# ImIntheMiddle/VATL4Pose-WACV2024

Measured on AMD Instinct MI355X. Metric: frames/sec pose-infer+uncertainty, 256x192 17-kp, higher is better.
Workload: dtype f32; 1 GPU; SimpleBaseline-R50 256x192 inference + decode + local-peak + THC-L1, 1024-frame synthetic video per GPU; frames_per_gpu=1024, batch=1024, tracks=4, parallelism=frame-sharded x1

## Files before the change

include/vatl_hip.h:

```cpp
#ifndef VATL_HIP_H
#define VATL_HIP_H

#include <stdint.h>

#ifdef __cplusplus
extern "C" {
#endif

#define VATL_VERSION 100
#define VATL_EINVAL  (-1)
#define VATL_ELAUNCH (-2)

int         vatl_version(void);
const char* vatl_last_error(void);

int vatl_flop_meter_begin(void);
int vatl_flop_meter_end(double* direct_flops, double* winograd_flops, int64_t* direct_launches, int64_t* winograd_launches);
#define VATL_ROUTE_NAMES "igemm,igemm_bnbwd,igemm_dma,persistent_1x1,streamk,rows_1x1,bottleneck_chain,stem_pool,halo_3x3," \
                         "winograd,winograd_2h,winograd_bnbwd,winograd_persist,winograd_c32,wgrad,winograd_wgrad,winograd_wgrad_2h," \
                         "winograd_wgrad_table,winograd_f4,winograd_f4_bnbwd,gemm1x1_ring"
int vatl_flop_meter_routes(int64_t* counts, int n);


int vatl_nchw_to_nhwc(const float* src, float* dst, int N, int C, int H, int W, int Cpad, void* stream);
int vatl_nhwc_to_nchw(const float* src, float* dst, int N, int C, int H, int W, void* stream);

int vatl_pack_conv_weight(const float* w_oihw, float* w_packed, int Cout, int Cin, int R, int S,
                          int CoutPad, int Spad, int CinPad, void* stream);
int vatl_pack_deconv4x4s2_weight(const float* w_iohw, float* w_packed, int Cin, int Cout, int CoutPad, void* stream);
int64_t vatl_stem_pool_weight_floats(void);
int vatl_pack_stem_pool_weight(const float* w_oihw, float* packed, void* stream);
int vatl_stem_pool_supported(int H, int W);
int vatl_stem7x7s2_pool_fwd(const float* x_nchw, const float* w_packed, const float* scale, const float* bias, float* y_nhwc,
                            int N, int H, int W, void* stream);
int64_t vatl_stem3_weight_floats(void);
int vatl_pack_stem3_weight(const float* w_oihw, float* packed, void* stream);
int vatl_stem3x3s2_fwd(const float* x_nchw, const float* w_packed, const float* scale, const float* bias, float* y_nhwc,
                       int N, int H, int W, void* stream);

int vatl_bn_fold(const float* gamma, const float* beta, const float* mean, const float* var, const float* conv_bias,
                 float eps, float* scale, float* bias, int C, void* stream);


// ... 230 lines not shown
```

vatl4pose-wacv2024_amd/csrc/common.h:

```cpp
#pragma once
#include <hip/hip_runtime.h>
#include <atomic>
#include <cstdarg>
#include <cstdio>
#include <cstdint>

#include "vatl_hip.h"

namespace vatl {

char* err_buf();
int fail(int code, const char* fmt, ...);

void meter_add(int kind, double flops);
enum MeterRoute {
    kRouteIgemm = 0, kRouteIgemmBnBwd, kRouteIgemmDma, kRoutePersistent1x1, kRouteStreamK, kRouteRows, kRouteChain, kRouteStemPool, kRouteHalo,
    kRouteWino, kRouteWino2H, kRouteWinoBnBwd, kRouteWinoPersist, kRouteWinoC32, kRouteWgrad, kRouteWinoWgrad, kRouteWinoWgrad2H,
    kRouteWinoWgradTable, kRouteWinoF4, kRouteWinoF4BnBwd, kRouteGemm1x1Ring, kRouteCount
};
void meter_route(int route);

inline int check_launch(const char* what) {
    hipError_t e = hipGetLastError();
    if (e != hipSuccess) return fail(VATL_ELAUNCH, "%s: %s", what, hipGetErrorString(e));
    return 0;
}

inline int ensure_dynamic_lds(const void* kern, int bytes, std::atomic<unsigned>& done_mask, const char* what) {
    int d = 0;
    if (hipGetDevice(&d) != hipSuccess) return fail(VATL_ELAUNCH, "%s: no current device", what);
    const unsigned bit = 1u << (d & 31);
    if (done_mask.load(std::memory_order_acquire) & bit) return 0;
    hipError_t e = hipFuncSetAttribute(kern, hipFuncAttributeMaxDynamicSharedMemorySize, bytes);
    if (e != hipSuccess) return fail(VATL_ELAUNCH, "hipFuncSetAttribute(%s): %s", what, hipGetErrorString(e));
    done_mask.fetch_or(bit, std::memory_order_release);
    return 0;
}

static inline int cdiv(int64_t a, int64_t b) { return (int)((a + b - 1) / b); }

typedef float f32x4 __attribute__((ext_vector_type(4)));
// ... 46 lines not shown
```

vatl4pose-wacv2024_amd/csrc/conv_igemm.hip:

```cpp
#include "common.h"

#include <algorithm>
#include <atomic>
#include <cstdlib>

namespace vatl {

struct ConvParams {
    const float* x;
    const float* w;
    const float* scale;
    const float* bias;
    const float* res;
    float* y;
    int N, H, W, Cin;
    int Cout, CoutPad;
    int R, S, stride, pad_y, pad_x;
    int Ho, Wo, M;
    int OH, OW, osy, osx, ooy, oox;
    int relu, out_nchw, deconv;
    int kpr;
    int ktiles;
    int n_tiles, m_tiles;
    int order;
// ... 1584 lines not shown
    if (bn == 64) {
        if (var == 2) return launch<128, 64, 64, 32, false, 2>(p, phases, st);
        if (var == 0) return launch<128, 64, 64, 32, false, 0>(p, phases, st);
        return launch<128, 64, 64, 32, false, 4>(p, phases, st);
    }
    if (var == 2) return launch<128, 32, 32, 32, false, 2>(p, phases, st);
    if (var == 0 || p.ktiles < 4) return launch<128, 32, 32, 32, false, 0>(p, phases, st);
    return launch<128, 32, 32, 32, false, 4>(p, phases, st);
}

}

namespace vatl {
int conv3x3_halo_try(const float* x, const float* w, const float* scale, const float* bias, const float* residual, float* y, int N, int H, int W,
                     int Cin, int Cout, int CoutPad, int R, int S, int stride, int pad, int relu, hipStream_t st);
int conv3x3_halo_enable(int on);
int wino_set_ablate(int bits);
int wino_set_group_kb(int v);
int wino_set_halves(int v);
int wino_set_persist(int v);
int wino_wgrad_set_halves(int v);
int wino_wgrad_set_table(int v);
int wino_set_persist_pf(int v);
int wino_wgrad_set_blocks(int v);

}

using namespace vatl;

namespace vatl {
__attribute__((visibility("hidden"))) int tune_wgrad_blocks(int blocks);
__attribute__((visibility("hidden"))) int crop_tune_px(int px);
}

extern "C" int vatl_tune_set(int knob, int value) {
    switch (knob) {
    case 0:  if (value == 0 || value == 2 || value == 4 || value == 5) { g_var.store(value, std::memory_order_relaxed); return 0; } break;
    case 1:  if (value == 0 || value == 1) { g_order.store(value, std::memory_order_relaxed); return 0; } break;
    case 5:  if (value == 0 || value == 64 || value == 128) { g_bm.store(value, std::memory_order_relaxed); return 0; } break;
    case 7:  if (value >= 0 && value <= 64) { g_persist.store(value, std::memory_order_relaxed); return 0; } break;
    case 8:  if (value == 0 || value == 1) return conv3x3_halo_enable(value); break;
    case 10: if (value == 1 || value == 2) { g_persist_dist.store(value, std::memory_order_relaxed); return 0; } break;
    case 18: if (value >= 0 && value <= (1 << 20)) return wino_set_group_kb(value); break;
    case 21: if (value >= 1 && value <= 3) return wino_set_halves(value); break;
    case 22: if (value >= 0 && value <= 4096) return wino_set_persist(value); break;
    case 24: if (value >= 0 && value <= 3) return wino_set_persist_pf(value); break;
    case 25: if (value == 0 || value == 1) return wino_wgrad_set_table(value); break;
    default: break;
    }
#ifdef VATL_ABLATION
    const bool wrong = (knob == 0 && value >= 10) || ((knob == 4 || knob == 6 || knob == 17) && value != 0);
    if (wrong) {
        const char* ok = getenv("VATL_ALLOW_ABLATION");
        if (!ok || ok[0] != '1') return fail(VATL_EINVAL, "tune_set: knob %d value %d is a profiling ablation (wrong results); set VATL_ALLOW_ABLATION=1", knob, value);
    }
    if (knob == 0 && value >= 10 && value <= 13) { g_var.store(value, std::memory_order_relaxed); return 0; }
    if (knob == 2 && value >= 0 && value <= 200) { g_stagger.store(value, std::memory_order_relaxed); return 0; }
    if (knob == 3 && tune_wgrad_blocks(value) == 0) return 0;
    if (knob == 4 && value >= 0 && value <= 3) return tune_wgrad_blocks(-value - 1);
    if (knob == 6 && value >= 0 && value <= 15) { g_ablate.store(value, std::memory_order_relaxed); return 0; }
    if (knob == 9 && (value == 0 || value == 1)) { g_splitk_policy.store(value, std::memory_order_relaxed); return 0; }
    if (knob == 12 && (value == 0 || value == 1)) { g_streamk.store(value, std::memory_order_relaxed); return 0; }
    if (knob == 16 && crop_tune_px(value) == 0) return 0;
    if (knob == 17 && value >= 0 && value <= 63) return wino_set_ablate(value);
    if (knob == 19 && value >= 1 && value <= (1 << 20)) return wino_wgrad_set_blocks(value);
    if (knob == 23 && value >= 1 && value <= 2) return wino_wgrad_set_halves(value);
    if (knob == 27 && (value == 0 || value == 1)) { g_ring.store(value, std::memory_order_relaxed); return 0; }
    return fail(VATL_EINVAL, "tune_set: unknown knob %d / value %d", knob, value);
#else
    return fail(VATL_EINVAL, "tune_set: knob %d / value %d is not a product knob (include/vatl_hip.h lists them: 0, 1, 5, 7, 8, 10, 18, 21, 22, 24, 25 — all bit-identical); "
                "knobs that change the summation order, performance experiments and profiling ablations exist only in the variant built with "
                "`build.py --ablation` (-DVATL_ABLATION)", knob, value);
#endif
}

extern "C" int vatl_set_splitk_workspace_thread(float* workspace, int64_t floats) {
    if (workspace && floats <= 0) return fail(VATL_EINVAL, "set_splitk_workspace_thread: empty workspace");
    tl_splitk_ws = workspace;
    tl_splitk_floats = workspace ? (long long)floats : 0;
    return 0;
}

extern "C" int64_t vatl_streamk_workspace_bytes(void) { return kStreamKBytes; }

extern "C" int vatl_set_streamk_workspace_thread(void* workspace, int64_t bytes) {
    if (workspace && bytes < kStreamKBytes) return fail(VATL_EINVAL, "set_streamk_workspace_thread: %lld bytes, need %lld", (long long)bytes, kStreamKBytes);
    tl_streamk_ws = static_cast<char*>(workspace);
    return 0;
}

// ... 164 lines not shown
```

vatl4pose-wacv2024_amd/csrc/conv_winograd.hip:

```cpp
#include "common.h"
#include "winograd_pack.h"

#include <algorithm>
#include <atomic>

namespace vatl {

struct WinoParams {
    const float* x;
    const float* u;
    const float* scale;
    const float* bias;
    const float* res;
    float* y;
    double* stats;
    const float* bz;
    const float* bmy;
    const float* bsc;
    const float* bbi;
    const float* bmu;
    const float* bis;
    int N, H, W, Cin, Cout;
    int TH, TW, tpi, Mtiles;
    int m_tiles, n_tiles;
    int relu;
    int stages;
    int nhp;
    int pad_y, pad_x;
    int OH, OW, os, ooy, oox;
    int deconv;
    int gather;
    int spp;
    int rn;
    int pg, periods, chunk;
    long long x_period_floats, y_period_floats;
    long long u_phase_floats;
    float neg_one;
    int ablate;
    unsigned x_bytes, u_bytes, y_bytes;
    FastDivU d_TH, d_TW, d_tpi, d_grp, d_rn, d_rn_last, d_ntiles;
};

constexpr unsigned WOOB_BASE = 0xF0000000u;
constexpr unsigned WOOB = 0xFFFFFFFFu;
constexpr unsigned WOOB_G = 0xFFFF0000u;
typedef unsigned int wu32x4 __attribute__((ext_vector_type(4)));

__device__ __forceinline__ f32x4 wbuf_load4(__amdgpu_buffer_rsrc_t r, unsigned byte_off) {
    return __builtin_bit_cast(f32x4, __builtin_amdgcn_raw_buffer_load_b128(r, byte_off, 0, 0));
}
__device__ __forceinline__ void wbuf_store4(__amdgpu_buffer_rsrc_t r, unsigned byte_off, f32x4 v) {
    __builtin_amdgcn_raw_buffer_store_b128(__builtin_bit_cast(wu32x4, v), r, byte_off, 0, 0);
}

constexpr int W_TB = 32;
constexpr int W_CK = 16;
constexpr int W_NQ = W_TB + 1;
constexpr int W_ZERO = 16;
constexpr int W_LDP = 32;
template <int MO> struct WinoStage {
    static constexpr int ROWE = MO * W_NQ + 1;
    static constexpr int ITEMS = 4 * ROWE * 4;
    static constexpr int NDMA = (ITEMS + 63) / 64;
    static constexpr int FLOATS = NDMA * 256;
    static constexpr int NLD = (NDMA + 3) / 4;
};

typedef __attribute__((address_space(3))) void wlds_void;

template <int MO, bool BNB, bool GATHER, int NB>
__device__ __forceinline__ void winograd_body(const WinoParams& p, float* smem, const int bid, const int nblk) {
    constexpr int NT = 256, BN = 32 * NB, NW = 4;
    using ST = WinoStage<MO>;
    constexpr int W_NLD = ST::NLD, STAGE = ST::FLOATS, ROWF = ST::ROWE * W_CK;
    float* Rs = smem + W_ZERO;

    int tid_ = threadIdx.x;
    if constexpr (GATHER) asm volatile("" : "+v"(tid_));
    const int tid = tid_, lane = tid & 63, xi = __builtin_amdgcn_readfirstlane(tid >> 6);

    const int xcd = bid & 7, loc = bid >> 3, q8 = nblk >> 3, r8 = nblk & 7;
    const int t = (xcd < r8 ? xcd * (q8 + 1) : r8 * (q8 + 1) + (xcd - r8) * q8) + loc;
    const int units = p.n_tiles * (p.deconv ? 4 : 1);
    const int grp = fdiv(t, p.d_grp), rem = t - grp * (p.m_tiles * p.rn);
    const bool last_grp = units - grp * p.rn < p.rn;
    const int rn_g = last_grp ? units - grp * p.rn : p.rn;
    const int m_tile = fdiv(rem, last_grp ? p.d_rn_last : p.d_rn), unit = grp * p.rn + (rem - m_tile * rn_g);
    const int phase = fdiv(unit, p.d_ntiles), n_tile = unit - phase * p.n_tiles;
    const int m0 = m_tile * W_TB, n0 = n_tile * BN;

    int pad_y = p.pad_y, pad_x = p.pad_x, ooy = p.ooy, oox = p.oox;
    const float* ubase_ptr = p.u;
    if (p.deconv) {
        const int py = phase >> 1, px = phase & 1;
        pad_y = 1 - py; pad_x = 1 - px; ooy = py; oox = px;
        ubase_ptr += (long long)phase * p.u_phase_floats;
    }
    const __amdgpu_buffer_rsrc_t xr = __builtin_amdgcn_make_buffer_rsrc(const_cast<float*>(p.x), 0, p.x_bytes, 0x00020000);
    const __amdgpu_buffer_rsrc_t ur = __builtin_amdgcn_make_buffer_rsrc(const_cast<float*>(ubase_ptr), 0, p.u_bytes, 0x00020000);

#ifdef VATL_ABLATION
    const int abl = p.ablate;
#else
    constexpr int abl = 0;
#endif
    constexpr bool EARLY = !GATHER;
    f32x4 ua[4], ub[4];
    if constexpr (EARLY) {
        const int hn0 = n_tile * NB, ut0 = hn0 / p.nhp;
        const unsigned u0 = (unsigned)((((ut0 * p.stages * 2) * 16 + 4 * xi) * p.nhp + (hn0 - ut0 * p.nhp)) * 64 + lane) << 4;
#pragma unroll
        for (int nu = 0; nu < 4; ++nu) ua[nu] = wbuf_load4(ur, (abl & 4) ? WOOB : u0 + nu * (p.nhp * 1024u));
    }

    unsigned goff[W_NLD];
    auto set_goff = [&](int ph) {
        const int gy = ph >> 1, gx = ph & 1;
        const int py_ = GATHER ? gy : pad_y, px_ = GATHER ? gx : pad_x;
#pragma unroll
        for (int u = 0; u < W_NLD; ++u) {
            const int pz = (xi + NW * u) * 64 + lane;
            goff[u] = WOOB_G;
            if (pz >= ST::ITEMS) continue;
            const int cpos = pz & 3, e = pz >> 2;
            const int i = e / ST::ROWE, re = e - i * ST::ROWE;
            const int r = re / W_NQ, q = re - r * W_NQ;
            if (r >= MO) continue;
            const int chunk = cpos ^ ((q >> 2) & 3);
            int m = m0 + q;
            int gr = fdiv(m, p.d_TW), tx = m - gr * p.TW;
            int xx = MO * tx + r - px_;
            if (m >= p.Mtiles || (tx == 0 && xx < 0)) {
                m -= 1;
                if (m < 0) continue;
                gr = fdiv(m, p.d_TW); tx = m - gr * p.TW;
// ... 50 lines not shown
    const float sgn = xi == 1 ? 1.f : -1.f;
    const f32x4 m1 = {p.neg_one, p.neg_one, p.neg_one, p.neg_one};
    const int roa = ia * ROWF, rob = ib * ROWF;

    const int steps = p.stages * 2;
    const int hn = n_tile * NB;
    const int ut = hn / p.nhp, nh_g = hn - ut * p.nhp;
    const int usteps = GATHER ? 2 * p.spp : steps;
    const unsigned ubase = (unsigned)((((ut * usteps) * 16 + 4 * xi) * p.nhp + nh_g) * 64 + lane) << 4;
    const unsigned ustep = 16u * p.nhp * 1024u, unu = p.nhp * 1024u;
    const unsigned uphase = (unsigned)(p.u_phase_floats * 4);
    auto u_load = [&](f32x4 (&dst)[4], int step_) {
        const int step = min(step_, steps - 1);
        unsigned off = ubase + (unsigned)step * ustep;
        if constexpr (GATHER) {
            const int ph = step / (2 * p.spp);
            off = ubase + (unsigned)ph * uphase + (unsigned)(step - ph * 2 * p.spp) * ustep;
        }
        if (abl & 4) off = WOOB_BASE;
#pragma unroll
        for (int nu = 0; nu < 4; ++nu) dst[nu] = wbuf_load4(ur, off + nu * unu);
    };

    f32x16 accs[NB][4];
#pragma unroll
    for (int hh = 0; hh < NB; ++hh)
#pragma unroll
        for (int nu = 0; nu < 4; ++nu)
#pragma unroll
            for (int e = 0; e < 16; ++e) accs[hh][nu][e] = 0.f;
    f32x16 (&acc)[4] = accs[0];

    if constexpr (!EARLY) {
        if (tid < W_ZERO / 4) *reinterpret_cast<f32x4*>(&smem[tid * 4]) = f32x4{0.f, 0.f, 0.f, 0.f};
        stage_dma(0, 0);
        u_load(ua, 0);
    }
    asm volatile("s_waitcnt vmcnt(0)" ::: "memory");
    __syncthreads();

    auto make_v = [&](f32x4 (&v)[4], const float* Rb, int x8, int pv) {
        f32x4 tc[4];
        if (abl & 2) {
#pragma unroll
            for (int j = 0; j < 4; ++j) tc[j] = f32x4{1.f + j, 2.f, 3.f, 4.f + x8};
        } else {
#pragma unroll
            for (int j = 0; j < 4; ++j) {
                const int a = ra[GATHER ? pv : 0][j];
// ... 5 lines not shown
                    continue;
                }
#endif
                const f32x4 da = *reinterpret_cast<const f32x4*>(Rb + roa + (a ^ x8));
                const f32x4 db = *reinterpret_cast<const f32x4*>(Rb + rob + (a ^ x8));
                tc[j] = da + sgn * db;
            }
        }
        v[0] = tc[0] + m1 * tc[2]; v[1] = tc[1] + tc[2]; v[2] = tc[2] + m1 * tc[1]; v[3] = tc[1] + m1 * tc[3];
    };
    auto mfma_group = [&](f32x16 (&ac)[4], const f32x4 (&v)[4], const f32x4 (&uu)[4]) {
#pragma unroll
        for (int tt = 0; tt < 4; ++tt)
#pragma unroll
            for (int nu = 0; nu < 4; ++nu)
                ac[nu] = __builtin_amdgcn_mfma_f32_32x32x2f32(v[nu][tt], uu[nu][tt], ac[nu], 0, 0, 0);
    };
    auto step_mfma = [&](const float* Rb, int x8, const f32x4 (&uu)[4], int pv) {
        f32x4 v[4];
        make_v(v, Rb, x8, pv);
        mfma_group(acc, v, uu);
    };

    if constexpr (NB == 2) {
        constexpr bool V_AHEAD = !GATHER && (MO == 2 || !BNB);
        auto u_load_h = [&](f32x4 (&dst)[4], int step_, int half) {
            const int step = min(step_, steps - 1);
            unsigned off = ubase + (unsigned)half * 1024u + (unsigned)step * ustep;
            if constexpr (GATHER) {
                const int ph = step / (2 * p.spp);
                off = ubase + (unsigned)half * 1024u + (unsigned)ph * uphase + (unsigned)(step - ph * 2 * p.spp) * ustep;
            }
            if (abl & 4) off = WOOB_BASE;
#pragma unroll
            for (int nu = 0; nu < 4; ++nu) dst[nu] = wbuf_load4(ur, off + nu * unu);
        };
        for (int st = 0; st < p.stages; ++st) {
            const int buf = st & 1;
            const float* Rb = Rs + buf * STAGE;
            const int pv = GATHER ? (st / p.spp) & 1 : 0;
            f32x4 v[4], v1[4];
            u_load_h(ub, 2 * st, 1);
            __builtin_amdgcn_sched_barrier(0);
            make_v(v, Rb, 0, pv);
            mfma_group(accs[0], v, ua);
            if constexpr (V_AHEAD) make_v(v1, Rb, 8, pv);
            __builtin_amdgcn_sched_barrier(0);
// ... 33 lines not shown
        __builtin_amdgcn_sched_barrier(0);
        step_mfma(Rb, 8, ub, pv);
        __builtin_amdgcn_sched_barrier(0);
        if (!(abl & 16)) {
            asm volatile("s_waitcnt vmcnt(0)" ::: "memory");
            __syncthreads();
        }
    }

#ifdef VATL_ABLATION
    if (abl & 16) __syncthreads();
    if (abl & 1) {
        float sacc = 0.f;
#pragma unroll
        for (int nu = 0; nu < 4; ++nu)
#pragma unroll
            for (int e = 0; e < 16; ++e) sacc += acc[nu][e];
        if (sacc == 12345.678f) p.y[0] = sacc;
        return;
    }
#endif
    constexpr int C4 = 32 / 4;
#pragma unroll
    for (int hh = 0; hh < NB; ++hh) {
        const int n0h = n0 + 32 * hh;
        f32x16 (&acch)[4] = accs[hh];
        f32x4 ssum = {0.f, 0.f, 0.f, 0.f}, ssq = {0.f, 0.f, 0.f, 0.f};
        const __amdgpu_buffer_rsrc_t yr = __builtin_amdgcn_make_buffer_rsrc(p.y, 0, p.y_bytes, 0x00020000);
        const __amdgpu_buffer_rsrc_t rr = __builtin_amdgcn_make_buffer_rsrc(const_cast<float*>(p.res), 0, p.res ? p.y_bytes : 0u, 0x00020000);
        const __amdgpu_buffer_rsrc_t zr = __builtin_amdgcn_make_buffer_rsrc(const_cast<float*>(BNB ? p.bz : p.x), 0, BNB ? p.y_bytes : 0u, 0x00020000);
        const __amdgpu_buffer_rsrc_t mr = __builtin_amdgcn_make_buffer_rsrc(const_cast<float*>(BNB ? p.bmy : p.x), 0, (BNB && p.bmy) ? p.y_bytes : 0u, 0x00020000);
        const int c4 = tid % C4;
        const int n = n0h + c4 * 4;
        const bool nv = n < p.Cout;
        const f32x4 one = {1.f, 1.f, 1.f, 1.f}, nul = {0.f, 0.f, 0.f, 0.f};
        const float lo = p.relu ? 0.f : -INFINITY;
        f32x4 sc = one, bi = nul, mu = nul, is = nul, msc = nul, mbi = one;
        auto request_consts = [&]() {
            if (nv && p.scale) sc = *reinterpret_cast<const f32x4*>(p.scale + n);
            if (nv && p.bias) bi = *reinterpret_cast<const f32x4*>(p.bias + n);
            if (BNB && nv) {
                mu = *reinterpret_cast<const f32x4*>(p.bmu + n); is = *reinterpret_cast<const f32x4*>(p.bis + n);
                if (p.bsc) { msc = *reinterpret_cast<const f32x4*>(p.bsc + n); mbi = *reinterpret_cast<const f32x4*>(p.bbi + n); }
            }
        };
        unsigned off[MO][MO];
        f32x4 rs[MO][MO];
        constexpr bool EARLY_Z = BNB && MO == 2;
        f32x4 zq[EARLY_Z ? MO : 1][EARLY_Z ? MO : 1], yq[EARLY_Z ? MO : 1][EARLY_Z ? MO : 1];
        auto request_out = [&](const int u) {
        {
            const int rest = (tid + NT * u) / C4;
            const int tl = rest / MO, bq = rest - tl * MO;
            const int m = m0 + tl;
    #pragma unroll
            for (int a = 0; a < MO; ++a) off[u][a] = WOOB;
            if (nv && m < p.Mtiles) {
                const int b = fdiv(m, p.d_tpi), r = m - b * p.tpi;
                const int ty = fdiv(r, p.d_TW), tx = r - ty * p.TW;
                const int xx = MO * tx + bq;
                if (xx < p.W) {
    #pragma unroll
                    for (int a = 0; a < MO; ++a) {
                        const int yy = MO * ty + a;
                        if (yy < p.H) off[u][a] = (unsigned)(((b * p.OH + yy * p.os + ooy) * p.OW + xx * p.os + oox) * p.Cout + n) << 2;
                    }
                }
            }
    #pragma unroll
            for (int a = 0; a < MO; ++a) rs[u][a] = p.res ? wbuf_load4(rr, off[u][a]) : nul;
            if constexpr (EARLY_Z) {
    #pragma unroll
                for (int a = 0; a < MO; ++a) { zq[u][a] = wbuf_load4(zr, off[u][a]); yq[u][a] = p.bmy ? wbuf_load4(mr, off[u][a]) : nul; }
            }
        }
        };
        if constexpr (EARLY) {
            request_consts();
    #pragma unroll
            for (int u = 0; u < MO; ++u) request_out(u);
            __builtin_amdgcn_sched_barrier(0);
        }

        float* Ps = smem;
        {
            const int cl = lane & 31;
    #pragma unroll
            for (int e = 0; e < 16; ++e) {
// ... 65 lines not shown
            lds_barrier();
            f32x4* sh = reinterpret_cast<f32x4*>(smem);
            sh[tid] = ssum; sh[NT + tid] = ssq;
            lds_barrier();
            if (tid < C4) {
                double ds[4] = {0, 0, 0, 0}, dq[4] = {0, 0, 0, 0};
    #pragma unroll 2
                for (int k = 0; k < NT / C4; ++k) {
                    const f32x4 a = sh[k * C4 + tid], b = sh[NT + k * C4 + tid];
    #pragma unroll
                    for (int c = 0; c < 4; ++c) { ds[c] += a[c]; dq[c] += b[c]; }
                }
                const long long rb = (long long)phase * p.m_tiles + m_tile;
    #pragma unroll
                for (int c = 0; c < 4; ++c) {
                    const int nn = n0h + tid * 4 + c;
                    if (nn < p.Cout) {
                        p.stats[(rb * p.Cout + nn) * 2 + 0] = ds[c];
                        p.stats[(rb * p.Cout + nn) * 2 + 1] = dq[c];
                    }
                }
            }
        }
        if (NB > 1 && hh + 1 < NB) lds_barrier();
    }
}

template <int NB, bool PF>
__device__ __forceinline__ void winograd_persist_body(const WinoParams& p, float* smem) {
    constexpr int MO = 2, NT = 256, BN = 32 * NB, NW = 4;
    using ST = WinoStage<MO>;
    constexpr int W_NLD = ST::NLD, STAGE = ST::FLOATS, ROWF = ST::ROWE * W_CK;
    float* Rs = smem + W_ZERO;
    const int tid = threadIdx.x, lane = tid & 63, xi = __builtin_amdgcn_readfirstlane(tid >> 6);

    const int bid = blockIdx.x, nblk = gridDim.x;
    const int xcd = bid & 7, loc = bid >> 3, q8 = nblk >> 3, r8 = nblk & 7;
    const int t = (xcd < r8 ? xcd * (q8 + 1) : r8 * (q8 + 1) + (xcd - r8) * q8) + loc;
    const int units = p.pg * p.n_tiles;
    const int part = fdiv(t, p.d_grp), unit = t - part * units;
    const int slot = fdiv(unit, p.d_ntiles), n_tile = unit - slot * p.n_tiles;
    const int it0 = part * p.chunk, it1 = min(it0 + p.chunk, p.periods);
    if (it0 >= it1) return;
    const int m0 = slot * W_TB, n0 = n_tile * BN;
    const int Lt = p.pg * W_TB;

    static_assert(W_NLD <= 5, "geometry record layout");
// ... 284 lines not shown
template <int NB, bool PF>
__global__ __launch_bounds__(256, (NB == 2 || PF) ? 2 : 3) void winograd_persist_kernel(WinoParams p) {
    extern __shared__ __attribute__((aligned(16))) float smem[];
    winograd_persist_body<NB, PF>(p, smem);
}

template <int MO, bool BNB, bool GATHER, int NB = 1>
__global__ __launch_bounds__(256, NB == 2 ? 2 : 3) void winograd_kernel(WinoParams p) {
    extern __shared__ __attribute__((aligned(16))) float smem[];
    if constexpr (GATHER) {
        typedef const __attribute__((address_space(4))) WinoParams* KArg;
        const int total = gridDim.x;
        for (int bid = blockIdx.x; bid < total; bid += gridDim.x) {
            KArg pp = (KArg)__builtin_amdgcn_kernarg_segment_ptr();
            asm volatile("" : "+s"(pp));
            winograd_body<MO, BNB, GATHER, NB>(*(const WinoParams*)pp, smem, bid, total);
            __syncthreads();
        }
    } else {
        winograd_body<MO, BNB, GATHER, NB>(p, smem, blockIdx.x, gridDim.x);
    }
}

__global__ __launch_bounds__(256) void wino_pack_kernel(const float* __restrict__ w, float* __restrict__ out, int Cout, int Cin, int NH, int mode, int w_i) {
    wino_pack_block(w, out, mode, w_i, Cout, Cin, NH, blockIdx.x, threadIdx.x);
}

static std::atomic<unsigned> g_wino_lds_done[12];
static std::atomic<int> g_wino_halves{2};
int wino_set_halves(int v) { g_wino_halves.store(v, std::memory_order_relaxed); return 0; }
static std::atomic<int> g_wino_ablate{0};
static std::atomic<int> g_wino_group_kb{2048};
int wino_set_group_kb(int v) { g_wino_group_kb.store(v, std::memory_order_relaxed); return 0; }
int wino_set_ablate(int bits) { g_wino_ablate.store(bits, std::memory_order_relaxed); return 0; }

static std::atomic<int> g_wino_persist{8};
int wino_set_persist(int v) { g_wino_persist.store(v, std::memory_order_relaxed); return 0; }
static std::atomic<unsigned> g_wino_persist_lds_done[4];
static std::atomic<int> g_wino_persist_pf{2};
int wino_set_persist_pf(int v) { g_wino_persist_pf.store(v, std::memory_order_relaxed); return 0; }

constexpr int kWinoMaxLds = 64 * 1024;

template <int MO, bool BNB, bool GATHER = false, int NB = 1>
static int launch_wino(const WinoParams& p, int phases, hipStream_t st) {
    auto kern = winograd_kernel<MO, BNB, GATHER, NB>;
    if (int rc = ensure_dynamic_lds((const void*)kern, kWinoMaxLds, g_wino_lds_done[(NB == 2 ? 6 : 0) + (GATHER ? 4 + (BNB ? 1 : 0) : (MO - 2) * 2 + (BNB ? 1 : 0))], "winograd")) return rc;
    const int loop = W_ZERO + 2 * WinoStage<MO>::FLOATS, epi = 4 * MO * W_TB * W_LDP, sta = 2 * 256 * 4;
    const int smem = std::max(loop, std::max(epi, sta)) * (int)sizeof(float);
    if (smem > kWinoMaxLds) return fail(VATL_EINVAL, "winograd: %d bytes of LDS per block", smem);
    hipLaunchKernelGGL(kern, dim3(p.m_tiles * p.n_tiles * phases), dim3(256), smem, st, p);
    meter_add(1, 2.0 * ((double)p.m_tiles * W_TB) * ((double)p.n_tiles * 32 * NB) * 16.0 * ((double)p.stages * W_CK) * phases);
    meter_route(BNB ? kRouteWinoBnBwd : (NB == 2 ? kRouteWino2H : kRouteWino));
    return check_launch("winograd");
}

static thread_local int tl_wino_route = 0;

static long long gcd_ll(long long a, long long b) { while (b) { const long long t = a % b; a = b; b = t; } return a; }

static int launch_wino_persist(const WinoParams& base, int N, bool two, hipStream_t st, int* covered) {
    *covered = 0;
    const int maxst = g_wino_persist.load(std::memory_order_relaxed);
    if (maxst <= 0 || base.stages > maxst || base.deconv || base.gather || base.stats || base.bz) return 0;
    const long long Lt = (long long)base.tpi / gcd_ll(base.tpi, W_TB) * W_TB;
    const int Pi = (int)(Lt / base.tpi), Pg = (int)(Lt / W_TB);
    const int periods = N / Pi;
    if (periods < 8 || Pg > 4096) return 0;
    const int NBh = two ? 2 : 1;
    const int n_tiles = cdiv(base.Cout, 32 * NBh);
    const int units = Pg * n_tiles, slots = (two || (g_wino_persist_pf.load(std::memory_order_relaxed) & 1)) ? 512 : 768;
    if (units > slots) return 0;
    int best_chunk = 0, best_parts = 0;
    double best_eff = 0.0;
    for (int k = 1; k <= 4; ++k) {
        const int np_max = std::min(periods, k * slots / units);
        if (np_max < 1) continue;
// ... 54 lines not shown

extern "C" int64_t vatl_winograd_deconv_weight_floats(int Cout, int Cin) { return 4 * vatl_winograd_weight_floats(Cout, Cin); }

extern "C" int vatl_pack_winograd_deconv_weight(const float* w, float* u, int Cout, int Cin, void* stream) {
    if (!w || !u || Cout <= 0 || Cin <= 0) return fail(VATL_EINVAL, "pack_winograd_deconv_weight: null pointer or empty filter");
    if (Cin % 16 != 0) return fail(VATL_EINVAL, "pack_winograd_deconv_weight: Cin %d must be a multiple of 16", Cin);
    const int pad = vatl_winograd_cout_pad(Cout);
    hipLaunchKernelGGL(wino_pack_kernel, dim3((unsigned)(4 * (pad / 32) * (Cin / 8))), dim3(256), 0, (hipStream_t)stream, w, u, Cout, Cin, wino_nh(Cout),
                       2, Cout);
    return check_launch("wino_pack_deconv");
}

struct WinoBn { const float *z, *mask_y, *scale, *bias, *mean, *invstd; };

static int winograd_impl(int MO, const float* x, const float* u, const float* scale, const float* bias, const float* residual, float* y,
                         double* stats, int64_t* row_blocks_used, int N, int H, int W, int Cin, int Cout, int relu, void* stream,
                         const WinoBn* fuse = nullptr, bool gather = false) {
    if (!x || !u || !y || N <= 0 || H <= 0 || W <= 0) return fail(VATL_EINVAL, "winograd: null pointer or empty batch");
    if (Cin % 16 != 0 || (Cout & 3)) return fail(VATL_EINVAL, "winograd: Cin %d must be a multiple of 16 and Cout %d of 4", Cin, Cout);
    WinoParams p{};
    p.neg_one = -1.0f;
    p.x = x; p.u = u; p.scale = scale; p.bias = bias; p.res = residual; p.y = y; p.stats = stats;
    p.N = N; p.H = H; p.W = W; p.Cin = Cin; p.Cout = Cout; p.relu = relu;
    p.TH = (H + MO - 1) / MO; p.TW = (W + MO - 1) / MO; p.tpi = p.TH * p.TW;
    const bool deconv = MO == 3 && !gather;
    const int phases = deconv ? 4 : 1, os = deconv ? 2 : 1;
    const long long mt = (long long)N * p.tpi, xe = (long long)N * H * W * Cin * (gather ? 4 : 1), ye = (long long)N * H * W * os * os * Cout;
    const long long ue = vatl_winograd_weight_floats(Cout, Cin);
    if (xe > (long long)(WOOB_G / 4) || ye >= (1LL << 30) || ue >= (1LL << 28) || mt >= (1LL << 30) || Cin / W_CK >= 1024)
        return fail(VATL_EINVAL, "winograd: a tensor exceeds 2^30 elements (32-bit buffer offsets); split the batch");
    p.Mtiles = (int)mt;
    p.nhp = wino_nh(Cout);
    p.spp = Cin / W_CK;
    p.stages = gather ? 4 * p.spp : p.spp;
    p.pad_y = 1; p.pad_x = 1; p.OH = H * os; p.OW = W * os; p.os = os; p.ooy = 0; p.oox = 0;
    p.deconv = deconv; p.gather = gather; p.u_phase_floats = ue;
    p.x_bytes = (unsigned)(xe * 4); p.y_bytes = (unsigned)(ye * 4); p.u_bytes = (unsigned)(ue * 4 * (gather ? 4 : 1));
    p.ablate = g_wino_ablate.load(std::memory_order_relaxed);
    p.m_tiles = cdiv(mt, W_TB);
    const int hv = g_wino_halves.load(std::memory_order_relaxed);
    const bool two = p.nhp == 2 && vatl_winograd_cout_pad(Cout) % 64 == 0 && hv >= 2 &&
                     (hv == 3 || (long long)p.m_tiles * cdiv(Cout, 64) * phases >= 400);
    const int NBh = two ? 2 : 1;
    p.n_tiles = cdiv(Cout, 32 * NBh);
    hipStream_t st = (hipStream_t)stream;
    if (MO == 2 && !fuse && !stats && !gather) {
        p.d_TH = make_fastdiv(p.TH); p.d_TW = make_fastdiv(p.TW); p.d_tpi = make_fastdiv(p.tpi);
        int covered = 0;
        if (int rc = launch_wino_persist(p, N, two, st, &covered)) return rc;
        tl_wino_route = covered == 0 ? 0 : (covered == N ? 1 : 2);
        if (covered == N) return 0;
        if (covered > 0) {
            const int rc = winograd_impl(MO, x + (long long)covered * H * W * Cin, u, scale, bias, residual ? residual + (long long)covered * H * W * Cout : nullptr,
                                 y + (long long)covered * H * W * Cout, nullptr, nullptr, N - covered, H, W, Cin, Cout, relu, stream);
            tl_wino_route = 2;
            return rc;
        }
    }
    if (row_blocks_used) *row_blocks_used = (int64_t)p.m_tiles * phases;
    const int gkb = g_wino_group_kb.load(std::memory_order_relaxed);
    p.rn = std::max(1, std::min(p.n_tiles * phases, std::max(gkb > 0 ? 2 : 1, gkb / (2 * Cin * NBh * (gather ? 4 : 1)))));
    const int units = p.n_tiles * phases;
    p.d_TH = make_fastdiv(p.TH); p.d_TW = make_fastdiv(p.TW); p.d_tpi = make_fastdiv(p.tpi);
    p.d_grp = make_fastdiv((unsigned)(p.m_tiles * p.rn)); p.d_rn = make_fastdiv(p.rn); p.d_ntiles = make_fastdiv(p.n_tiles);
    p.d_rn_last = make_fastdiv(units % p.rn ? units % p.rn : p.rn);
    if ((long long)p.m_tiles * units >= (1LL << 31)) return fail(VATL_EINVAL, "winograd: too many blocks");
    if (fuse) {
        if (deconv) return fail(VATL_EINVAL, "winograd: the BatchNorm-backward epilogue exists for the data-gradient launches only");
        p.bz = fuse->z; p.bmy = fuse->mask_y; p.bsc = fuse->scale; p.bbi = fuse->bias; p.bmu = fuse->mean; p.bis = fuse->invstd;
        if (gather) return two ? launch_wino<3, true, true, 2>(p, phases, st) : launch_wino<3, true, true>(p, phases, st);
        if (two) return MO == 2 ? launch_wino<2, true, false, 2>(p, phases, st) : launch_wino<3, true, false, 2>(p, phases, st);
        return MO == 2 ? launch_wino<2, true>(p, phases, st) : launch_wino<3, true>(p, phases, st);
    }
    if (gather) return two ? launch_wino<3, false, true, 2>(p, phases, st) : launch_wino<3, false, true>(p, phases, st);
    if (two) return MO == 2 ? launch_wino<2, false, false, 2>(p, phases, st) : launch_wino<3, false, false, 2>(p, phases, st);
    return MO == 2 ? launch_wino<2, false>(p, phases, st) : launch_wino<3, false>(p, phases, st);
}

extern "C" int vatl_conv3x3_winograd_fwd(const float* x, const float* u, const float* scale, const float* bias, const float* residual, float* y,
                                         int N, int H, int W, int Cin, int Cout, int relu, void* stream) {
    return winograd_impl(2, x, u, scale, bias, residual, y, nullptr, nullptr, N, H, W, Cin, Cout, relu, stream);
}

extern "C" int vatl_winograd_last_route(void) { return tl_wino_route; }

extern "C" int64_t vatl_winograd_stats_row_blocks(int64_t N, int H, int W) { return (N * ((H + 1) / 2) * ((W + 1) / 2) + W_TB - 1) / W_TB; }

extern "C" int vatl_conv3x3_winograd_fwd_stats(const float* x, const float* u, float* y, double* stats, int64_t* row_blocks_used, int N, int H,
                                               int W, int Cin, int Cout, void* stream) {
    if (!stats || !row_blocks_used) return fail(VATL_EINVAL, "conv3x3_winograd_fwd_stats: null statistics buffer");
    return winograd_impl(2, x, u, nullptr, nullptr, nullptr, y, stats, row_blocks_used, N, H, W, Cin, Cout, 0, stream);
}

extern "C" int vatl_conv3x3_winograd_fwd_bnbwd(const float* x, const float* u, const float* residual, float* y, int N, int H, int W, int Cin, int Cout,
                                               const float* bn_z, const float* bn_mask_y, const float* bn_scale, const float* bn_bias,
                                               const float* bn_mean, const float* bn_invstd, double* stats, int64_t* row_blocks_used, void* stream) {
    if (!bn_z || !stats || !row_blocks_used || !bn_mean || !bn_invstd || (bn_scale && !bn_bias))
// ... 44 lines not shown
```

vatl4pose-wacv2024_amd/vatl_hip/__init__.py:

```python
from __future__ import annotations

import ctypes as C
import os

import torch

_HERE = os.path.dirname(os.path.abspath(__file__))
LIB_PATH = os.environ.get("VATL_HIP_LIB") or os.path.join(_HERE, "libvatl_hip.so")

_p = C.c_void_p
_i = C.c_int
_f = C.c_float
_d = C.c_double
_i64 = C.c_int64

SIGNATURES = {
    "vatl_version": (_i, []),
    "vatl_last_error": (C.c_char_p, []),
    "vatl_flop_meter_begin": (_i, []),
    "vatl_flop_meter_end": (_i, [_p, _p, _p, _p]),
    "vatl_flop_meter_routes": (_i, [_p, _i]),
    "vatl_nchw_to_nhwc": (_i, [_p, _p, _i, _i, _i, _i, _i, _p]),
    "vatl_nhwc_to_nchw": (_i, [_p, _p, _i, _i, _i, _i, _p]),
    "vatl_pack_conv_weight": (_i, [_p, _p, _i, _i, _i, _i, _i, _i, _i, _p]),
# ... 175 lines not shown

def _stream():
    return torch.cuda.current_stream().cuda_stream



def nchw_to_nhwc(x: torch.Tensor, cpad: int | None = None) -> torch.Tensor:
    n, c, h, w = x.shape
    cpad = cpad or c
    y = torch.empty((n, h, w, cpad), device=x.device, dtype=torch.float32)
    _check(lib().vatl_nchw_to_nhwc(_ptr(x), _ptr(y), n, c, h, w, cpad, _stream()), "vatl_nchw_to_nhwc")
    return y


def nhwc_to_nchw(x: torch.Tensor) -> torch.Tensor:
    n, h, w, c = x.shape
    y = torch.empty((n, c, h, w), device=x.device, dtype=torch.float32)
    _check(lib().vatl_nhwc_to_nchw(_ptr(x), _ptr(y), n, c, h, w, _stream()), "vatl_nhwc_to_nchw")
    return y


ROUTE_NAMES = ("igemm", "igemm_bnbwd", "igemm_dma", "persistent_1x1", "streamk", "rows_1x1", "bottleneck_chain", "stem_pool", "halo_3x3", "winograd",
               "winograd_2h", "winograd_bnbwd", "winograd_persist", "winograd_c32", "wgrad", "winograd_wgrad", "winograd_wgrad_2h", "winograd_wgrad_table", "winograd_f4", "winograd_f4_bnbwd",
               "gemm1x1_ring")


class flop_meter:

    def __enter__(self):
        _check(lib().vatl_flop_meter_begin(), "flop_meter_begin")
        self.direct = self.winograd = self.total = 0.0
        self.direct_launches = self.winograd_launches = 0
        return self

    @staticmethod
    def launches_now() -> int:
        counts = (C.c_int64 * len(ROUTE_NAMES))()
        _check(min(0, lib().vatl_flop_meter_routes(counts, len(ROUTE_NAMES))), "flop_meter_routes")
        return int(sum(counts))

    def __exit__(self, *exc):
        counts = (C.c_int64 * len(ROUTE_NAMES))()
        _check(min(0, lib().vatl_flop_meter_routes(counts, len(ROUTE_NAMES))), "flop_meter_routes")
        self.routes = {n: int(c) for n, c in zip(ROUTE_NAMES, counts)}
        d, w, nd, nw = C.c_double(0), C.c_double(0), C.c_int64(0), C.c_int64(0)
        _check(lib().vatl_flop_meter_end(C.byref(d), C.byref(w), C.byref(nd), C.byref(nw)), "flop_meter_end")
        self.direct, self.winograd, self.total = d.value, w.value, d.value + w.value
# ... 1170 lines not shown
```

Measured before the change: 16490 frames/s.

## Add paired-phase Winograd kernel for 4x4 stride-2 deconv sharing input tiles

Adds a Winograd kernel for the transposed-conv (deconv) head that computes two vertical output phases per block from one staged input tile. A row shift makes both phases share the same input rows, so each block runs four filter sub-groups against one set of staged activations, halving input staging and tile-transform traffic per output. The kernel is enabled by default when the layer is large enough and the output height is not a multiple of three. In exchange it doubles accumulator registers, uses a launch bound of one block per CU, and adds a more complex filter-load pipeline that could lower occupancy.

```diff
diff --git a/include/vatl_hip.h b/include/vatl_hip.h
--- a/include/vatl_hip.h
+++ b/include/vatl_hip.h
@@ -18,7 +18,7 @@
 int vatl_flop_meter_end(double* direct_flops, double* winograd_flops, int64_t* direct_launches, int64_t* winograd_launches);
 #define VATL_ROUTE_NAMES "igemm,igemm_bnbwd,igemm_dma,persistent_1x1,streamk,rows_1x1,bottleneck_chain,stem_pool,halo_3x3," \
                          "winograd,winograd_2h,winograd_bnbwd,winograd_persist,winograd_c32,wgrad,winograd_wgrad,winograd_wgrad_2h," \
-                         "winograd_wgrad_table,winograd_f4,winograd_f4_bnbwd,gemm1x1_ring"
+                         "winograd_wgrad_table,winograd_f4,winograd_f4_bnbwd,gemm1x1_ring,winograd_pair"
 int vatl_flop_meter_routes(int64_t* counts, int n);
 
 
diff --git a/vatl4pose-wacv2024_amd/csrc/common.h b/vatl4pose-wacv2024_amd/csrc/common.h
--- a/vatl4pose-wacv2024_amd/csrc/common.h
+++ b/vatl4pose-wacv2024_amd/csrc/common.h
@@ -16,7 +16,7 @@
 enum MeterRoute {
     kRouteIgemm = 0, kRouteIgemmBnBwd, kRouteIgemmDma, kRoutePersistent1x1, kRouteStreamK, kRouteRows, kRouteChain, kRouteStemPool, kRouteHalo,
     kRouteWino, kRouteWino2H, kRouteWinoBnBwd, kRouteWinoPersist, kRouteWinoC32, kRouteWgrad, kRouteWinoWgrad, kRouteWinoWgrad2H,
-    kRouteWinoWgradTable, kRouteWinoF4, kRouteWinoF4BnBwd, kRouteGemm1x1Ring, kRouteCount
+    kRouteWinoWgradTable, kRouteWinoF4, kRouteWinoF4BnBwd, kRouteGemm1x1Ring, kRouteWinoPair, kRouteCount
 };
 void meter_route(int route);
 
diff --git a/vatl4pose-wacv2024_amd/csrc/conv_igemm.hip b/vatl4pose-wacv2024_amd/csrc/conv_igemm.hip
--- a/vatl4pose-wacv2024_amd/csrc/conv_igemm.hip
+++ b/vatl4pose-wacv2024_amd/csrc/conv_igemm.hip
@@ -1630,6 +1630,7 @@
 int wino_wgrad_set_halves(int v);
 int wino_wgrad_set_table(int v);
 int wino_set_persist_pf(int v);
+int wino_set_pair(int v);
 int wino_wgrad_set_blocks(int v);
 
 }
@@ -1674,6 +1675,7 @@
     if (knob == 19 && value >= 1 && value <= (1 << 20)) return wino_wgrad_set_blocks(value);
     if (knob == 23 && value >= 1 && value <= 2) return wino_wgrad_set_halves(value);
     if (knob == 27 && (value == 0 || value == 1)) { g_ring.store(value, std::memory_order_relaxed); return 0; }
+    if (knob == 28 && (value == 0 || value == 1)) return wino_set_pair(value);
     return fail(VATL_EINVAL, "tune_set: unknown knob %d / value %d", knob, value);
 #else
     return fail(VATL_EINVAL, "tune_set: knob %d / value %d is not a product knob (include/vatl_hip.h lists them: 0, 1, 5, 7, 8, 10, 18, 21, 22, 24, 25 — all bit-identical); "
diff --git a/vatl4pose-wacv2024_amd/csrc/conv_winograd.hip b/vatl4pose-wacv2024_amd/csrc/conv_winograd.hip
--- a/vatl4pose-wacv2024_amd/csrc/conv_winograd.hip
+++ b/vatl4pose-wacv2024_amd/csrc/conv_winograd.hip
@@ -29,6 +29,7 @@
     int pad_y, pad_x;
     int OH, OW, os, ooy, oox;
     int deconv;
+    int rowshift;
     int gather;
     int spp;
     int rn;
@@ -68,9 +69,11 @@
 
 typedef __attribute__((address_space(3))) void wlds_void;
 
-template <int MO, bool BNB, bool GATHER, int NB>
+template <int MO, bool BNB, bool GATHER, int NB, bool PAIR = false>
 __device__ __forceinline__ void winograd_body(const WinoParams& p, float* smem, const int bid, const int nblk) {
     constexpr int NT = 256, BN = 32 * NB, NW = 4;
+    constexpr int NP = PAIR ? 2 : 1;
+    static_assert(!PAIR || (MO == 3 && NB == 2 && !BNB && !GATHER), "the pair block is the forward transposed conv with two filter halves");
     using ST = WinoStage<MO>;
     constexpr int W_NLD = ST::NLD, STAGE = ST::FLOATS, ROWF = ST::ROWE * W_CK;
     float* Rs = smem + W_ZERO;
@@ -81,7 +84,7 @@
 
     const int xcd = bid & 7, loc = bid >> 3, q8 = nblk >> 3, r8 = nblk & 7;
     const int t = (xcd < r8 ? xcd * (q8 + 1) : r8 * (q8 + 1) + (xcd - r8) * q8) + loc;
-    const int units = p.n_tiles * (p.deconv ? 4 : 1);
+    const int units = p.n_tiles * (PAIR ? 2 : (p.deconv ? 4 : 1));
     const int grp = fdiv(t, p.d_grp), rem = t - grp * (p.m_tiles * p.rn);
     const bool last_grp = units - grp * p.rn < p.rn;
     const int rn_g = last_grp ? units - grp * p.rn : p.rn;
@@ -89,13 +92,14 @@
     const int phase = fdiv(unit, p.d_ntiles), n_tile = unit - phase * p.n_tiles;
     const int m0 = m_tile * W_TB, n0 = n_tile * BN;
 
-    int pad_y = p.pad_y, pad_x = p.pad_x, ooy = p.ooy, oox = p.oox;
+    int pad_y = p.pad_y, pad_x = p.pad_x, ooy = p.ooy, oox = p.oox, sy = 0;
     const float* ubase_ptr = p.u;
     if (p.deconv) {
         const int py = phase >> 1, px = phase & 1;
-        pad_y = 1 - py; pad_x = 1 - px; ooy = py; oox = px;
+        pad_y = p.rowshift ? 1 : 1 - py; pad_x = 1 - px; ooy = py; oox = px; sy = p.rowshift ? py : 0;
         ubase_ptr += (long long)phase * p.u_phase_floats;
     }
+    const unsigned upy = (unsigned)(2 * p.u_phase_floats * 4);
     const __amdgpu_buffer_rsrc_t xr = __builtin_amdgcn_make_buffer_rsrc(const_cast<float*>(p.x), 0, p.x_bytes, 0x00020000);
     const __amdgpu_buffer_rsrc_t ur = __builtin_amdgcn_make_buffer_rsrc(const_cast<float*>(ubase_ptr), 0, p.u_bytes, 0x00020000);
 
@@ -106,11 +110,19 @@
 #endif
     constexpr bool EARLY = !GATHER;
     f32x4 ua[4], ub[4];
+    f32x4 fs[PAIR ? 4 : 1][4];
     if constexpr (EARLY) {
         const int hn0 = n_tile * NB, ut0 = hn0 / p.nhp;
         const unsigned u0 = (unsigned)((((ut0 * p.stages * 2) * 16 + 4 * xi) * p.nhp + (hn0 - ut0 * p.nhp)) * 64 + lane) << 4;
-#pragma unroll
-        for (int nu = 0; nu < 4; ++nu) ua[nu] = wbuf_load4(ur, (abl & 4) ? WOOB : u0 + nu * (p.nhp * 1024u));
+        if constexpr (PAIR) {
+#pragma unroll
+            for (int g = 0; g < 3; ++g)
+#pragma unroll
+                for (int nu = 0; nu < 4; ++nu) fs[g][nu] = wbuf_load4(ur, (abl & 4) ? WOOB : u0 + (g >> 1) * upy + (g & 1) * 1024u + nu * (p.nhp * 1024u));
+        } else {
+#pragma unroll
+            for (int nu = 0; nu < 4; ++nu) ua[nu] = wbuf_load4(ur, (abl & 4) ? WOOB : u0 + nu * (p.nhp * 1024u));
+        }
     }
 
     unsigned goff[W_NLD];
@@ -207,9 +219,9 @@
         for (int nu = 0; nu < 4; ++nu) dst[nu] = wbuf_load4(ur, off + nu * unu);
     };
 
-    f32x16 accs[NB][4];
-#pragma unroll
-    for (int hh = 0; hh < NB; ++hh)
+    f32x16 accs[NP * NB][4];
+#pragma unroll
+    for (int hh = 0; hh < NP * NB; ++hh)
 #pragma unroll
         for (int nu = 0; nu < 4; ++nu)
 #pragma unroll
@@ -261,7 +273,39 @@
         mfma_group(acc, v, uu);
     };
 
-    if constexpr (NB == 2) {
+    if constexpr (PAIR) {
+        auto u_load_g = [&](f32x4 (&dst)[4], int grp_) {
+            const int step = min(grp_ >> 2, steps - 1), sub = grp_ & 3;
+            unsigned off = ubase + (unsigned)(sub >> 1) * upy + (unsigned)(sub & 1) * 1024u + (unsigned)step * ustep;
+            if (abl & 4) off = WOOB_BASE;
+#pragma unroll
+            for (int nu = 0; nu < 4; ++nu) dst[nu] = wbuf_load4(ur, off + nu * unu);
+        };
+        for (int st = 0; st < p.stages; ++st) {
+            const int buf = st & 1;
+            const float* Rb = Rs + buf * STAGE;
+            f32x4 v[4], v1[4];
+            make_v(v, Rb, 0, 0);
+#pragma unroll
+            for (int j = 0; j < 8; ++j) {
+                u_load_g(fs[(j + 3) & 3], 8 * st + j + 3);
+                __builtin_amdgcn_sched_barrier(0);
+                if (j == 0 && st + 1 < p.stages && st > 0 && !(abl & 8)) stage_dma(buf ^ 1, st + 1);
+                __builtin_amdgcn_sched_barrier(0);
+                if (j == 4) {
+#pragma unroll
+                    for (int nu = 0; nu < 4; ++nu) v[nu] = v1[nu];
+                }
+                mfma_group(accs[j & 3], v, fs[j & 3]);
+                if (j == 0) make_v(v1, Rb, 8, 0);
+                __builtin_amdgcn_sched_barrier(0);
+            }
+            if (!(abl & 16)) {
+                asm volatile("s_waitcnt vmcnt(28)" ::: "memory");
+                __syncthreads();
+            }
+        }
+    } else if constexpr (NB == 2) {
         constexpr bool V_AHEAD = !GATHER && (MO == 2 || !BNB);
         auto u_load_h = [&](f32x4 (&dst)[4], int step_, int half) {
             const int step = min(step_, steps - 1);
@@ -341,9 +385,11 @@
 #endif
     constexpr int C4 = 32 / 4;
 #pragma unroll
-    for (int hh = 0; hh < NB; ++hh) {
+    for (int gq = 0; gq < NP * NB; ++gq) {
+        const int hh = gq % NB;
+        const int syg = PAIR ? gq / NB : sy, ooyg = PAIR ? gq / NB : ooy;
         const int n0h = n0 + 32 * hh;
-        f32x16 (&acch)[4] = accs[hh];
+        f32x16 (&acch)[4] = accs[gq];
         f32x4 ssum = {0.f, 0.f, 0.f, 0.f}, ssq = {0.f, 0.f, 0.f, 0.f};
         const __amdgpu_buffer_rsrc_t yr = __builtin_amdgcn_make_buffer_rsrc(p.y, 0, p.y_bytes, 0x00020000);
         const __amdgpu_buffer_rsrc_t rr = __builtin_amdgcn_make_buffer_rsrc(const_cast<float*>(p.res), 0, p.res ? p.y_bytes : 0u, 0x00020000);
@@ -381,8 +427,8 @@
                 if (xx < p.W) {
     #pragma unroll
                     for (int a = 0; a < MO; ++a) {
-                        const int yy = MO * ty + a;
-                        if (yy < p.H) off[u][a] = (unsigned)(((b * p.OH + yy * p.os + ooy) * p.OW + xx * p.os + oox) * p.Cout + n) << 2;
+                        const int yy = MO * ty + a - syg;
+                        if ((unsigned)yy < (unsigned)p.H) off[u][a] = (unsigned)(((b * p.OH + yy * p.os + ooyg) * p.OW + xx * p.os + oox) * p.Cout + n) << 2;
                     }
                 }
             }
@@ -494,7 +540,7 @@
                 }
             }
         }
-        if (NB > 1 && hh + 1 < NB) lds_barrier();
+        if (gq + 1 < NP * NB) lds_barrier();
     }
 }
 
@@ -825,11 +871,18 @@
     }
 }
 
+__global__ __launch_bounds__(256, 1) void winograd_pair_kernel(WinoParams p) {
+    extern __shared__ __attribute__((aligned(16))) float smem[];
+    winograd_body<3, false, false, 2, true>(p, smem, blockIdx.x, gridDim.x);
+}
+
 __global__ __launch_bounds__(256) void wino_pack_kernel(const float* __restrict__ w, float* __restrict__ out, int Cout, int Cin, int NH, int mode, int w_i) {
     wino_pack_block(w, out, mode, w_i, Cout, Cin, NH, blockIdx.x, threadIdx.x);
 }
 
-static std::atomic<unsigned> g_wino_lds_done[12];
+static std::atomic<unsigned> g_wino_lds_done[13];
+static std::atomic<int> g_wino_pair{1};
+int wino_set_pair(int v) { g_wino_pair.store(v, std::memory_order_relaxed); return 0; }
 static std::atomic<int> g_wino_halves{2};
 int wino_set_halves(int v) { g_wino_halves.store(v, std::memory_order_relaxed); return 0; }
 static std::atomic<int> g_wino_ablate{0};
@@ -856,6 +909,16 @@
     meter_add(1, 2.0 * ((double)p.m_tiles * W_TB) * ((double)p.n_tiles * 32 * NB) * 16.0 * ((double)p.stages * W_CK) * phases);
     meter_route(BNB ? kRouteWinoBnBwd : (NB == 2 ? kRouteWino2H : kRouteWino));
     return check_launch("winograd");
+}
+
+static int launch_wino_pair(const WinoParams& p, hipStream_t st) {
+    if (int rc = ensure_dynamic_lds((const void*)winograd_pair_kernel, kWinoMaxLds, g_wino_lds_done[12], "winograd_pair")) return rc;
+    const int loop = W_ZERO + 2 * WinoStage<3>::FLOATS, epi = 4 * 3 * W_TB * W_LDP;
+    const int smem = std::max(loop, epi) * (int)sizeof(float);
+    hipLaunchKernelGGL(winograd_pair_kernel, dim3(p.m_tiles * p.n_tiles * 2), dim3(256), smem, st, p);
+    meter_add(1, 2.0 * ((double)p.m_tiles * W_TB) * ((double)p.n_tiles * 64) * 16.0 * ((double)p.stages * W_CK) * 4);
+    meter_route(kRouteWinoPair);
+    return check_launch("winograd_pair");
 }
 
 static thread_local int tl_wino_route = 0;
@@ -956,8 +1019,9 @@
     p.neg_one = -1.0f;
     p.x = x; p.u = u; p.scale = scale; p.bias = bias; p.res = residual; p.y = y; p.stats = stats;
     p.N = N; p.H = H; p.W = W; p.Cin = Cin; p.Cout = Cout; p.relu = relu;
+    const bool deconv = MO == 3 && !gather;
     p.TH = (H + MO - 1) / MO; p.TW = (W + MO - 1) / MO; p.tpi = p.TH * p.TW;
-    const bool deconv = MO == 3 && !gather;
+    p.rowshift = deconv && H % 3 != 0;
     const int phases = deconv ? 4 : 1, os = deconv ? 2 : 1;
     const long long mt = (long long)N * p.tpi, xe = (long long)N * H * W * Cin * (gather ? 4 : 1), ye = (long long)N * H * W * os * os * Cout;
     const long long ue = vatl_winograd_weight_floats(Cout, Cin);
@@ -972,9 +1036,13 @@
     p.x_bytes = (unsigned)(xe * 4); p.y_bytes = (unsigned)(ye * 4); p.u_bytes = (unsigned)(ue * 4 * (gather ? 4 : 1));
     p.ablate = g_wino_ablate.load(std::memory_order_relaxed);
     p.m_tiles = cdiv(mt, W_TB);
+    constexpr long long kPairMinBlocks = 1024;
+    constexpr int kPairMinStages = 128;
+    const bool pair = deconv && p.rowshift && !stats && !fuse && p.spp >= kPairMinStages && g_wino_pair.load(std::memory_order_relaxed) != 0 && p.nhp == 2 &&
+                      vatl_winograd_cout_pad(Cout) % 64 == 0 && (long long)p.m_tiles * cdiv(Cout, 64) * 2 >= kPairMinBlocks;
     const int hv = g_wino_halves.load(std::memory_order_relaxed);
-    const bool two = p.nhp == 2 && vatl_winograd_cout_pad(Cout) % 64 == 0 && hv >= 2 &&
-                     (hv == 3 || (long long)p.m_tiles * cdiv(Cout, 64) * phases >= 400);
+    const bool two = pair || (p.nhp == 2 && vatl_winograd_cout_pad(Cout) % 64 == 0 && hv >= 2 &&
+                              (hv == 3 || (long long)p.m_tiles * cdiv(Cout, 64) * phases >= 400));
     const int NBh = two ? 2 : 1;
     p.n_tiles = cdiv(Cout, 32 * NBh);
     hipStream_t st = (hipStream_t)stream;
@@ -993,8 +1061,9 @@
     }
     if (row_blocks_used) *row_blocks_used = (int64_t)p.m_tiles * phases;
     const int gkb = g_wino_group_kb.load(std::memory_order_relaxed);
-    p.rn = std::max(1, std::min(p.n_tiles * phases, std::max(gkb > 0 ? 2 : 1, gkb / (2 * Cin * NBh * (gather ? 4 : 1)))));
-    const int units = p.n_tiles * phases;
+    const int uphases = pair ? 2 : phases;
+    p.rn = std::max(1, std::min(p.n_tiles * uphases, std::max(gkb > 0 ? 2 : 1, gkb / (2 * Cin * NBh * (gather ? 4 : 1) * (pair ? 2 : 1)))));
+    const int units = p.n_tiles * uphases;
     p.d_TH = make_fastdiv(p.TH); p.d_TW = make_fastdiv(p.TW); p.d_tpi = make_fastdiv(p.tpi);
     p.d_grp = make_fastdiv((unsigned)(p.m_tiles * p.rn)); p.d_rn = make_fastdiv(p.rn); p.d_ntiles = make_fastdiv(p.n_tiles);
     p.d_rn_last = make_fastdiv(units % p.rn ? units % p.rn : p.rn);
@@ -1007,6 +1076,10 @@
         return MO == 2 ? launch_wino<2, true>(p, phases, st) : launch_wino<3, true>(p, phases, st);
     }
     if (gather) return two ? launch_wino<3, false, true, 2>(p, phases, st) : launch_wino<3, false, true>(p, phases, st);
+    if (pair) {
+        p.u_bytes = (unsigned)(ue * 4 * 3);
+        return launch_wino_pair(p, st);
+    }
     if (two) return MO == 2 ? launch_wino<2, false, false, 2>(p, phases, st) : launch_wino<3, false, false, 2>(p, phases, st);
     return MO == 2 ? launch_wino<2, false>(p, phases, st) : launch_wino<3, false>(p, phases, st);
 }
diff --git a/vatl4pose-wacv2024_amd/vatl_hip/__init__.py b/vatl4pose-wacv2024_amd/vatl_hip/__init__.py
--- a/vatl4pose-wacv2024_amd/vatl_hip/__init__.py
+++ b/vatl4pose-wacv2024_amd/vatl_hip/__init__.py
@@ -221,7 +221,7 @@
 
 ROUTE_NAMES = ("igemm", "igemm_bnbwd", "igemm_dma", "persistent_1x1", "streamk", "rows_1x1", "bottleneck_chain", "stem_pool", "halo_3x3", "winograd",
                "winograd_2h", "winograd_bnbwd", "winograd_persist", "winograd_c32", "wgrad", "winograd_wgrad", "winograd_wgrad_2h", "winograd_wgrad_table", "winograd_f4", "winograd_f4_bnbwd",
-               "gemm1x1_ring")
+               "gemm1x1_ring", "winograd_pair")
 
 
 class flop_meter:
```

After: 16470 frames/s, median of 2. About the same (-0.1%).
